# radiocosmology/driftscan

Measured on AMD Instinct MI355X. Metric: m-blocks/sec (BT-gen + SVD + KL), higher is better.
Workload: dtype f64; 1 GPU; configs[1]: 32-feed unpolarised cylinder, nfreq=16, nbase=46, lmax=mmax=128, 129 m-blocks per GPU per step, KLTransform with foregrounds; nfreq=16, nbase=46, lmax=128, mmax=128, sht_iter=3, mode=weak, ranks=1

## Files before the change

### driftscan_amd/_lib.py

```python
import ctypes
import os

import numpy as np

_HERE = os.path.dirname(os.path.abspath(__file__))
LIBPATH = os.path.join(_HERE, "lib", "libdriftmi.so")
if os.environ.get("DRIFTMI_LIB"):
    LIBPATH = os.environ["DRIFTMI_LIB"]

c_int = ctypes.c_int
c_i64 = ctypes.c_int64
c_dbl = ctypes.c_double
c_vp = ctypes.c_void_p
c_sz = ctypes.c_size_t

class ZgemmProblem(ctypes.Structure):
    _fields_ = [("A", c_vp), ("B", c_vp), ("C", c_vp), ("M", c_int), ("N", c_int), ("K", c_int),
                ("rsA", c_int), ("csA", c_int), ("rsB", c_int), ("csB", c_int), ("ldc", c_int),
                ("conjA", c_int), ("conjB", c_int), ("alpha", c_dbl), ("beta", c_dbl)]


class ZgemmProblemEx(ctypes.Structure):
    _fields_ = [("A", c_vp), ("B", c_vp), ("C", c_vp), ("kscale", c_vp), ("bgather", c_vp),
                ("M", c_int), ("N", c_int), ("K", c_int),
# ... 44 lines not shown
        c_int,
        [c_vp, c_int, c_int, c_int, c_dbl, c_vp, c_int, c_int, c_int, c_i64, c_vp, c_int, c_int, c_int, c_i64,
         c_dbl, c_vp, c_int, c_i64, c_vp, c_i64, c_int],
    ),
    "dm_zgemm_grouped": (c_int, [c_vp, c_int, ctypes.POINTER(ZgemmProblem)]),
    "dm_zgemm_grouped_ex": (c_int, [c_vp, c_int, ctypes.POINTER(ZgemmProblemEx)]),
    "dm_zgemm_plan_info": (c_int, [c_int, ctypes.POINTER(ZgemmProblemEx), c_int, ctypes.POINTER(ZgemmLaunchInfo),
                                   ctypes.POINTER(c_int)]),
    "dm_zpotrf_batched": (c_int, [c_vp, c_int, c_vp, c_int, c_i64, c_int, ctypes.POINTER(c_int)]),
    "dm_ztrsm_left_lower_batched": (
        c_int, [c_vp, c_int, c_int, c_vp, c_int, c_i64, c_vp, c_int, c_i64, c_int, c_int]),
    "dm_zpotrf_problems": (c_int, [c_vp, c_int, ctypes.POINTER(ZpotrfProblem), ctypes.POINTER(c_int)]),
    "dm_ztrsm_problems": (c_int, [c_vp, c_int, ctypes.POINTER(ZtrsmProblem), c_int, c_int]),
    "dm_zpotrf_problems_check": (c_int, [c_int, ctypes.POINTER(ZpotrfProblem)]),
    "dm_ztrsm_problems_check": (c_int, [c_int, ctypes.POINTER(ZtrsmProblem), c_int, c_int]),
    "dm_jacobi_rows_batched": (
        c_int, [c_vp, c_int, c_int, c_int, c_int, c_vp, c_int, c_i64, c_int, c_vp, ctypes.POINTER(c_int)]),
    "dm_jacobi_rows_problems": (
        c_int, [c_vp, c_int, ctypes.POINTER(JacobiProblemDesc), c_vp, c_int, ctypes.POINTER(JacobiOptions),
                ctypes.POINTER(c_int)]),
    "dm_jacobi_herm_batched": (
        c_int, [c_vp, c_int, c_vp, c_int, c_i64, c_vp, c_int, c_i64, c_int, c_vp, ctypes.POINTER(c_int)]),
    "dm_herm_eig_batched": (c_int, [c_vp, c_int, c_vp, c_int, c_i64, c_vp, c_int, c_i64, c_int, c_vp]),
    "dm_svd_chain": (
        c_int, [c_vp, c_int, c_int, c_int, c_int, c_int, c_vp, c_vp, c_dbl, c_vp, c_vp, c_vp, c_vp,
                ctypes.POINTER(c_int), ctypes.POINTER(c_int)]),
    "dm_svd_chain_lmin": (
        c_int, [c_vp, c_int, c_int, c_int, c_int, c_int, ctypes.POINTER(c_int), c_vp, c_vp, c_dbl, c_vp, c_vp, c_vp, c_vp,
                ctypes.POINTER(c_int), ctypes.POINTER(c_int)]),
    "dm_project_cov": (
# ... 392 lines not shown
        self.check(self.lib.dm_zpotrf_problems(self.h, n, _zpotrf_records(problems, ptrs), info), "dm_zpotrf_problems")
        return np.array(info[:n], dtype=np.int64)

    def ztrsm_problems(self, problems, conjtrans=False, upper_only=False):
        ptrs = []
        for p in problems:
            self._c128_device(p["L"], "ztrsm_problems")
            self._c128_device(p["B"], "ztrsm_problems")
            ztrsm_check_views(p, int(p["L"].numel()), int(p["B"].numel()))
            full = int(p["n"]) > 0 and int(p["nrhs"]) > 0
            ptrs.append((p["L"].data_ptr() + 16 * int(p.get("l_off", 0)) if full else 0,
                         p["B"].data_ptr() + 16 * int(p.get("b_off", 0)) if full else 0))
        self.check(self.lib.dm_ztrsm_problems(self.h, len(problems), _ztrsm_records(problems, ptrs),
                                              int(bool(conjtrans)), int(bool(upper_only))), "dm_ztrsm_problems")

    def jacobi_rows(self, Z, rows, cols, gc0, gc1, ld, stride=0, batch=1):
        sigma = self.empty((batch, max(rows, 1)), np.float64)
        sw = c_int(0)
        self.check(self.lib.dm_jacobi_rows_batched(self.h, rows, cols, gc0, gc1, self.ptr(Z), ld, stride, batch,
                                                   self.ptr(sigma), ctypes.byref(sw)), "dm_jacobi_rows_batched")
        return sigma, sw.value

    def jacobi_rows_problems(self, Z, problems, sigma=None, sigma_stride=None, **opts):
        n = len(problems)
        unknown = set(opts) - {f[0] for f in JacobiOptions._fields_}
        if unknown:
            raise ValueError("jacobi_rows_problems: unknown option(s) %s" % sorted(unknown))
        if n and not (Z.is_complex() and Z.element_size() == 16 and Z.is_contiguous()):
            raise ValueError("jacobi_rows_problems: a contiguous complex128 device tensor expected")
        arr = (JacobiProblemDesc * max(n, 1))()
# ... 1049 lines not shown
```

### driftscan_amd/csrc/dm_api.hip

```cpp
#include "dm_common.h"
#include "dm_kernels.h"
#include "../../include/driftmi.h"

#include <algorithm>

extern "C" {

int dm_zgemm_strided_batched(dm_ctx* ctx, int M, int N, int K, double alpha, const void* A, int rsA, int csA,
                             int conjA, int64_t strideA, const void* B, int rsB, int csB, int conjB,
                             int64_t strideB, double beta, void* C, int ldc, int64_t strideC,
                             const double* kscale, int64_t stride_kscale, int batch) {
  if (!ctx) return DM_EARG;
  DM_ARG(ctx, M >= 0 && N >= 0 && K >= 0 && batch >= 0 && A && B && C);
  dm_ws_scope ws_scope__(ctx);
  const size_t mark = ws_scope__.mark;
  std::vector<dm_gemm_desc> g;
  g.reserve(batch);
  for (int b = 0; b < batch; ++b) {
    g.push_back(dm_gemm_make(reinterpret_cast<const cplx*>(A) + b * strideA, rsA, csA, conjA != 0,
                             reinterpret_cast<const cplx*>(B) + b * strideB, rsB, csB, conjB != 0,
                             reinterpret_cast<cplx*>(C) + b * strideC, ldc, M, N, K, alpha, beta,
                             kscale ? kscale + b * stride_kscale : nullptr));
  }
  int rc = dm_gemm_grouped_launch(ctx, g);
// ... 189 lines not shown
  DM_TRY(dm_potrf_batched(ctx, mats, info_dev));
  return dm_download(ctx, info_host, info_dev, sizeof(int) * nprob);
}

int dm_ztrsm_problems(dm_ctx* ctx, int nprob, const dm_ztrsm_problem* probs, int conjtrans, int upper_only) {
  if (!ctx) return DM_EARG;
  DM_ARG(ctx, dm_ztrsm_problems_check(nprob, probs, conjtrans, upper_only) == DM_OK);
  dm_ws_scope ws_scope__(ctx);
  std::vector<dm_trsm_problem> ps(nprob);
  for (int i = 0; i < nprob; ++i)
    ps[i] = dm_trsm_problem{reinterpret_cast<const cplx*>(probs[i].L), probs[i].ldl, probs[i].n,
                            reinterpret_cast<cplx*>(probs[i].B), probs[i].ldb, probs[i].nrhs};
  return dm_trsm_left_lower_batched(ctx, ps, conjtrans != 0, upper_only != 0);
}

int dm_jacobi_rows_batched(dm_ctx* ctx, int rows, int cols, int gc0, int gc1, void* Z, int ld, int64_t stride,
                           int batch, double* sigma_dev, int* sweeps_host) {
  if (!ctx) return DM_EARG;
  DM_ARG(ctx, rows >= 0 && cols >= 0 && gc0 >= 0 && gc1 <= cols && gc0 <= gc1 && Z && sigma_dev && batch >= 0);
  std::vector<dm_jac_problem> ps(batch);
  for (int b = 0; b < batch; ++b)
    ps[b] = dm_jac_problem{reinterpret_cast<cplx*>(Z) + b * stride, ld, 0, rows, cols, gc0, gc1};
  return dm_jacobi_rows(ctx, ps, sigma_dev, rows > 0 ? rows : 1, sweeps_host);
}

int dm_jacobi_rows_problems(dm_ctx* ctx, int nprob, const dm_jacobi_problem_desc* probs, double* sigma_dev,
                            int sigma_stride, const dm_jacobi_options* opts, int* sweeps_host) {
  if (!ctx) return DM_EARG;
  DM_ARG(ctx, nprob >= 0 && (nprob == 0 || (probs && sigma_dev)) && sigma_stride >= 0);
  std::vector<dm_jac_problem> ps(nprob);
// ... 43 lines not shown
```

### driftscan_amd/csrc/dm_chol.hip

```cpp
#include "dm_common.h"
#include "dm_kernels.h"

#include <algorithm>

namespace {

constexpr int NB = 32;

struct chol_desc {
  cplx* A; int ld; int n;
};

__global__ __launch_bounds__(256) void potf2_kernel(const chol_desc* __restrict__ ds, int k0, int* __restrict__ info) {
  __shared__ cplx T[NB][NB + 1];
  __shared__ cplx Lo[NB][NB + 1];
  const chol_desc d = ds[blockIdx.x];
  if (k0 >= d.n) return;
  if (info[blockIdx.x] != 0) return;
  const int nb = min(NB, d.n - k0);
  const int tid = threadIdx.x;
  for (int idx = tid; idx < NB * NB; idx += 256) {
    int r = idx / NB, c = idx % NB;
    T[r][c] = (r < nb && c < nb && c <= r) ? d.A[(size_t)(k0 + r) * d.ld + k0 + c] : make_double2(0.0, 0.0);
    Lo[r][c] = make_double2(0.0, 0.0);
// ... 118 lines not shown
#pragma unroll
    for (int rr = 0; rr < NB; ++rr) {
      const int r = NB - 1 - rr;
      if (r < nb) {
        x[r] = cscale(x[r], 1.0 / Lk[r][r].x);
#pragma unroll
        for (int j = 0; j < r; ++j) x[j] = csub(x[j], cmul(cconj(Lk[r][j]), x[r]));
      }
    }
  }
#pragma unroll
  for (int r = 0; r < NB; ++r)
    if (r < nb) d.B[(size_t)(k0 + r) * d.ldb + col] = x[r];
}

}

int dm_potrf_batched(dm_ctx* ctx, const std::vector<dm_mat>& mats, int* info_dev) {
  const int nbatch = (int)mats.size();
  if (nbatch == 0) return DM_OK;
  dm_ws_scope ws_scope__(ctx);
  const size_t mark = ws_scope__.mark;
  std::vector<chol_desc> ds(nbatch);
  int maxn = 0;
  for (int i = 0; i < nbatch; ++i) {
    ds[i] = chol_desc{mats[i].p, mats[i].ld, mats[i].n};
    maxn = std::max(maxn, mats[i].n);
  }
  chol_desc* dd = dm_ws_upload(ctx, ds);
  if (!dd) return DM_ENOMEM;
  DM_HIP(ctx, hipMemsetAsync(info_dev, 0, sizeof(int) * nbatch, ctx->stream));
  if (maxn == 0) return DM_OK;
  dm_gemm_chain chain(ctx);
// ... 23 lines not shown
      const int k2 = k0 + 2 * NB;
      if (k2 < maxn) {
        DM_TRY(chain.gemm([&](std::vector<dm_gemm_desc>& g) {
          for (int i = 0; i < nbatch; ++i) {
            const int rem = mats[i].n - k2;
            if (rem <= 0) continue;
            cplx* L21 = mats[i].p + (size_t)k2 * mats[i].ld + k0;
            cplx* A22 = mats[i].p + (size_t)k2 * mats[i].ld + k2;
            g.push_back(dm_gemm_make(L21, mats[i].ld, 1, false, L21, 1, mats[i].ld, true, A22, mats[i].ld, rem, rem,
                                     2 * NB, -1.0, 1.0, nullptr, DM_GEMM_LOWER));
          }
        }));
      }
    }
  }
  DM_PLAUNCH(ctx, DM_PROF_CHOL, zero_upper_kernel, dim3((maxn + 255) / 256, maxn, nbatch), dim3(256), 0, ctx->stream, dd);
  DM_HIP(ctx, hipGetLastError());
  (void)mark;
  return DM_OK;
}

namespace {
int trsm_pass(dm_ctx* ctx, const std::vector<dm_trsm_problem>& probs, bool conjtrans, bool upper_only, dm_gemm_chain& chain,
              const trsm_desc* dd) {
  const int nbatch = (int)probs.size();
  int maxn = 0, maxrhs = 0;
  for (int i = 0; i < nbatch; ++i) {
    maxn = std::max(maxn, probs[i].n);
    maxrhs = std::max(maxrhs, probs[i].nrhs);
  }
  const int ct = (maxrhs + 255) / 256;
  const int NB2 = 2 * NB;
  const int nblk = (maxn + NB2 - 1) / NB2;
  const int nblk32 = (maxn + NB - 1) / NB;
  for (int s = 0; s < nblk; ++s) {
    DM_TRY(chain.gemm([&](std::vector<dm_gemm_desc>& g) {
    for (int i = 0; i < nbatch; ++i) {
      const dm_trsm_problem& P = probs[i];
      const int pn = (P.n + NB2 - 1) / NB2;
      if (!conjtrans) {
        if (s == 0 || s >= pn) continue;
        const int size = s & -s;
        const int r0 = s * NB2, r1 = std::min((s + size) * NB2, P.n);
        const int c0 = (s - size) * NB2;
        const int j0 = upper_only ? std::min(r0, P.nrhs) : 0;
        if (P.nrhs - j0 <= 0) continue;
        g.push_back(dm_gemm_make(P.L + (size_t)r0 * P.ldl + c0, P.ldl, 1, false, P.B + (size_t)c0 * P.ldb + j0, P.ldb, 1,
                                 false, P.B + (size_t)r0 * P.ldb + j0, P.ldb, r1 - r0, P.nrhs - j0, size * NB2, -1.0,
                                 1.0));
      } else {
        if (s < nblk - pn) continue;
        const int u = s - (nblk - pn);
        if (u == 0) continue;
        const int kb = pn - 1 - u;
        const int size = u & -u;
        const int t0 = std::max(kb - size + 1, 0) * NB2, t1 = (kb + 1) * NB2;
        const int k1 = t1, k2 = std::min((kb + 1 + size) * NB2, P.n);
        g.push_back(dm_gemm_make(P.L + (size_t)k1 * P.ldl + t0, 1, P.ldl, true, P.B + (size_t)k1 * P.ldb, P.ldb, 1,
                                 false, P.B + (size_t)t0 * P.ldb, P.ldb, t1 - t0, P.nrhs, k2 - k1, -1.0, 1.0));
      }
    }
    }));
    for (int half = 0; half < 2; ++half) {
      const int h = conjtrans ? 1 - half : half;
      int s32;
      if (!conjtrans) s32 = 2 * s + h;
      else s32 = 2 * s + half;
      if (chain.dry) {
      } else if (!conjtrans)
        DM_PLAUNCH(ctx, DM_PROF_CHOL, diag_solve_kernel<false>, dim3(ct, nbatch), dim3(256), 0, ctx->stream, dd, s32, nblk32,
                           upper_only ? 1 : 0);
      else
        DM_PLAUNCH(ctx, DM_PROF_CHOL, diag_solve_kernel<true>, dim3(ct, nbatch), dim3(256), 0, ctx->stream, dd, s32, 2 * nblk, 0);
      if (half == 0) {
        DM_TRY(chain.gemm([&](std::vector<dm_gemm_desc>& g2) {
        for (int i = 0; i < nbatch; ++i) {
          const dm_trsm_problem& P = probs[i];
          const int pn = (P.n + NB2 - 1) / NB2;
          if (!conjtrans) {
            const int k0 = s * NB2, k1 = k0 + NB;
            if (k1 >= P.n) continue;
            const int nb = std::min(NB, P.n - k1);
            const int j0 = upper_only ? std::min(k0, P.nrhs) : 0;
            if (P.nrhs - j0 <= 0) continue;
            g2.push_back(dm_gemm_make(P.L + (size_t)k1 * P.ldl + k0, P.ldl, 1, false, P.B + (size_t)k0 * P.ldb + j0,
                                      P.ldb, 1, false, P.B + (size_t)k1 * P.ldb + j0, P.ldb, nb, P.nrhs - j0, NB, -1.0,
                                      1.0));
          } else {
            if (s < nblk - pn) continue;
            const int kb = pn - 1 - (s - (nblk - pn));
            const int k0 = kb * NB2, k1 = k0 + NB;
            if (k1 >= P.n) continue;
            const int nb2 = std::min(NB, P.n - k1);
            g2.push_back(dm_gemm_make(P.L + (size_t)k1 * P.ldl + k0, 1, P.ldl, true, P.B + (size_t)k1 * P.ldb, P.ldb,
                                      1, false, P.B + (size_t)k0 * P.ldb, P.ldb, NB, P.nrhs, nb2, -1.0, 1.0));
          }
        }
        }));
      }
    }
  }
  return DM_OK;
}
}

int dm_trsm_plan_build(dm_ctx* ctx, const std::vector<dm_trsm_problem>& probs, bool conjtrans, bool upper_only, dm_trsm_plan& plan) {
  if (conjtrans) upper_only = false;
  if (upper_only)
    for (const auto& P : probs) DM_ARG(ctx, P.nrhs == P.n);
  plan.probs = probs;
  plan.conjtrans = conjtrans;
  plan.upper_only = upper_only;
  plan.chain.reset(new dm_gemm_chain(ctx));
  plan.empty = true;
  for (const auto& P : probs)
    if (P.n > 0 && P.nrhs > 0) plan.empty = false;
  if (plan.empty) return DM_OK;
  return trsm_pass(ctx, plan.probs, conjtrans, upper_only, *plan.chain, nullptr);
}

int dm_trsm_plan_run(dm_ctx* ctx, dm_trsm_plan& plan) {
  if (plan.empty || !plan.chain) return DM_OK;
  const int nbatch = (int)plan.probs.size();
  std::vector<trsm_desc> ds(nbatch);
  for (int i = 0; i < nbatch; ++i)
    ds[i] = trsm_desc{plan.probs[i].L, plan.probs[i].ldl, plan.probs[i].n, plan.probs[i].B, plan.probs[i].ldb, plan.probs[i].nrhs};
  trsm_desc* dd = dm_ws_upload(ctx, ds);
  if (!dd) return DM_ENOMEM;
  DM_TRY(plan.chain->upload());
  DM_TRY(trsm_pass(ctx, plan.probs, plan.conjtrans, plan.upper_only, *plan.chain, dd));
  DM_HIP(ctx, hipGetLastError());
  return DM_OK;
}

int dm_trsm_left_lower_batched(dm_ctx* ctx, const std::vector<dm_trsm_problem>& probs, bool conjtrans, bool upper_only) {
  dm_trsm_plan plan;
  DM_TRY(dm_trsm_plan_build(ctx, probs, conjtrans, upper_only, plan));
  return dm_trsm_plan_run(ctx, plan);
}
```

### driftscan_amd/csrc/dm_kernels.h

```cpp
#pragma once

#include "dm_common.h"

#include <deque>
#include <memory>
#include <functional>

enum {
  DM_GEMM_CONJ_A = 1,
  DM_GEMM_CONJ_B = 2,
  DM_GEMM_B_REAL = 4,
  DM_GEMM_LOWER = 8,
  DM_GEMM_ALL_REAL = 16,
  DM_GEMM_UPPER = 32,
  DM_GEMM_UPPER128 = 128,
  DM_GEMM_B_GATHER = 64,
};

struct dm_gemm_desc {
  const void* A;
  const void* B;
  void* C;
  const double* kscale;
  const int2* bgather;
// ... 95 lines not shown
                   int* sweeps_out = nullptr);

struct dm_eig_select {
  std::function<void(int p, const double* ev, int n, std::vector<int>& cols)> pick;
  std::vector<int> nsel;
};
int dm_herm_eig_tridiag(dm_ctx* ctx, const std::vector<dm_jac_herm_problem>& probs, double* evals, int evals_stride,
                        dm_eig_select* sel = nullptr, int two_stage = -1);

int dm_sort_rows_by_key(dm_ctx* ctx, const std::vector<dm_jac_problem>& probs, double* key, int key_stride,
                        bool descending);

struct dm_mat {
  cplx* p; int ld; int n;
};
int dm_potrf_batched(dm_ctx* ctx, const std::vector<dm_mat>& mats, int* info_dev);
struct dm_trsm_problem {
  const cplx* L; int ldl; int n;
  cplx* B; int ldb; int nrhs;
};
int dm_trsm_left_lower_batched(dm_ctx* ctx, const std::vector<dm_trsm_problem>& probs, bool conjtrans, bool upper_only = false);
struct dm_gemm_chain;
struct dm_trsm_plan {
  std::vector<dm_trsm_problem> probs;
  bool conjtrans = false, upper_only = false, empty = true;
  std::shared_ptr<dm_gemm_chain> chain;
};
int dm_trsm_plan_build(dm_ctx* ctx, const std::vector<dm_trsm_problem>& probs, bool conjtrans, bool upper_only, dm_trsm_plan& plan);
int dm_trsm_plan_run(dm_ctx* ctx, dm_trsm_plan& plan);

constexpr int DM_BAND_LC = 4;

struct dm_band_proj {
  int nblk = 0, F = 0, K = 0, P = 0, L = 0, R = 0;
  const int* svnum = nullptr;
  const int* nmodes = nullptr;
  const int64_t* evals_off = nullptr;
  std::vector<int> ndof, active, l0eff;
  std::vector<int64_t> off1;
  size_t tot1 = 0, totw = 0;
  int init(dm_ctx* ctx, int nblk_, int F_, int K_, int P_, int L_, const int* svnum_host, const int* l0_host,
           const int* nmodes_host, const int64_t* evals_off_host, int R_);
  int to_svd(dm_ctx* ctx, const cplx* evecs, const int64_t* evecs_off, const double* w, const int64_t* x_off, int nset,
// ... 21 lines not shown
```

### driftscan_amd/csrc/dm_kl.hip

```cpp
#include "dm_common.h"
#include "dm_kernels.h"
#include "../../include/driftmi.h"

#include <algorithm>
#include <chrono>
#include <cmath>

namespace {

struct blk_desc {
  cplx* a; int n;
};

constexpr int BLK_SPLIT = 16;

__device__ __forceinline__ bool lex_gt(double are, double aim, double bre, double bim) {
  return are > bre || (are == bre && aim > bim);
}

__global__ __launch_bounds__(256) void lexmax_partial_kernel(const blk_desc* __restrict__ bd, double2* __restrict__ part) {
  const blk_desc d = bd[blockIdx.y];
  __shared__ double sre[256], sim[256];
  double bre = -INFINITY, bim = -INFINITY;
  const size_t tot = (size_t)d.n * d.n;
// ... 43 lines not shown
  const size_t tot = (size_t)d.n * d.n;
  int mine = 0;
  for (size_t i = (size_t)blockIdx.x * 256 + threadIdx.x; i < tot; i += (size_t)BLK_SPLIT * 256) {
    cplx v = d.a[i];
    if (v.x != 0.0 || v.y != 0.0) mine = 1;
  }
  if (mine) flag[blockIdx.y] = 0;
}

__global__ void add_diag_kernel(const blk_desc* __restrict__ bd, const double* __restrict__ val) {
  const blk_desc d = bd[blockIdx.y];
  const int i = blockIdx.x * blockDim.x + threadIdx.x;
  if (i < d.n) d.a[(size_t)i * d.n + i].x += val[blockIdx.y];
}


int copy_async(dm_ctx* ctx, cplx* dst, const cplx* src, size_t n) {
  if (n == 0) return DM_OK;
  DM_HIP(ctx, hipMemcpyAsync(dst, src, n * sizeof(cplx), hipMemcpyDeviceToDevice, ctx->stream));
  return DM_OK;
}

}

extern "C" {

int dm_project_cov(dm_ctx* ctx, int nblk, int F, int K, int P, int L, const void* beam_svd_dev,
                   const int* svnum_host, const int* l0_host, const double* cl_pfl_dev, int npol,
                   const int* polmask_host, void* out_dev, const int64_t* out_off_host, int zero_first) {
  if (!ctx) return DM_EARG;
// ... 148 lines not shown
  cplx* E = reinterpret_cast<cplx*>(evecs_dev);

  size_t tot = 0;
  int maxn = 0;
  for (int b = 0; b < nblk; ++b) {
    tot += (size_t)n_host[b] * n_host[b];
    maxn = std::max(maxn, n_host[b]);
    add_const_host[b] = 0.0;
  }
  std::vector<size_t> loff(nblk);
  {
    size_t o = 0;
    for (int b = 0; b < nblk; ++b) { loff[b] = o; o += (size_t)n_host[b] * n_host[b]; }
  }
  cplx* Lw = dm_ws_alloc_t<cplx>(ctx, std::max<size_t>(tot, 1));
  cplx* Tw = dm_ws_alloc_t<cplx>(ctx, std::max<size_t>(tot, 1));
  cplx* Ww = dm_ws_alloc_t<cplx>(ctx, std::max<size_t>(tot, 1));
  double* evw = dm_ws_alloc_t<double>(ctx, (size_t)nblk * std::max(maxn, 1));
  int* info_dev = dm_ws_alloc_t<int>(ctx, nblk);
  int* zflag_dev = dm_ws_alloc_t<int>(ctx, nblk);
  if (!Lw || !Tw || !Ww || !evw || !info_dev || !zflag_dev) return DM_ENOMEM;

  std::vector<blk_desc> bdA(nblk);
  for (int b = 0; b < nblk; ++b) bdA[b] = blk_desc{A + off_host[b], n_host[b]};
  blk_desc* d_bdA = dm_ws_upload(ctx, bdA);
  if (!d_bdA) return DM_ENOMEM;
  DM_PLAUNCH(ctx, DM_PROF_UTIL, flag_set_kernel, dim3((nblk + 255) / 256), dim3(256), 0, ctx->stream, zflag_dev, nblk, 1);
  DM_PLAUNCH(ctx, DM_PROF_UTIL, allzero_kernel, dim3(BLK_SPLIT, nblk), dim3(256), 0, ctx->stream, d_bdA, zflag_dev);
  auto factor_launch = [&](const std::vector<int>& blks) -> int {
    std::vector<dm_mat> mats;
    std::vector<dm_cdesc> cp;
    for (int b : blks) {
      cp.push_back(dm_cdesc{B + off_host[b], Lw + loff[b], sizeof(cplx) * (size_t)n_host[b] * n_host[b]});
      mats.push_back(dm_mat{Lw + loff[b], n_host[b], n_host[b]});
    }
    DM_TRY(dm_copy_batched(ctx, cp));
    return dm_potrf_batched(ctx, mats, info_dev);
  };
  auto factor = [&](const std::vector<int>& blks, std::vector<int>& info) -> int {
    DM_TRY(factor_launch(blks));
    info.resize(blks.size());
    if (!blks.empty()) DM_TRY(dm_download(ctx, info.data(), info_dev, sizeof(int) * blks.size()));
    return DM_OK;
  };
  auto trsm_lists = [&](const std::vector<int>& blks, std::vector<dm_trsm_problem>& t1, std::vector<dm_trsm_problem>& t2) {
    t1.clear();
    t2.clear();
    for (int b : blks) {
      t1.push_back(dm_trsm_problem{Lw + loff[b], n_host[b], n_host[b], A + off_host[b], n_host[b], n_host[b]});
      t2.push_back(dm_trsm_problem{Lw + loff[b], n_host[b], n_host[b], Tw + loff[b], n_host[b], n_host[b]});
    }
  };
  std::vector<int> cand;
  for (int b = 0; b < nblk; ++b)
    if (n_host[b] > 0) cand.push_back(b);
  static const bool host_times = getenv("DM_TIME_HOST") != nullptr;
  const auto ht0 = std::chrono::steady_clock::now();
  DM_TRY(factor_launch(cand));
  const auto ht1 = std::chrono::steady_clock::now();
  dm_trsm_plan plan1, plan2;
  {
    std::vector<dm_trsm_problem> t1, t2;
    trsm_lists(cand, t1, t2);
    DM_TRY(dm_trsm_plan_build(ctx, t1, false, false, plan1));
    DM_TRY(dm_trsm_plan_build(ctx, t2, false, true, plan2));
  }
  const auto ht2 = std::chrono::steady_clock::now();
  std::vector<int> zflag(nblk);
  DM_TRY(dm_download(ctx, zflag.data(), zflag_dev, sizeof(int) * nblk));
  if (host_times) {
    const auto ht3 = std::chrono::steady_clock::now();
    auto ms = [](auto a, auto b) { return std::chrono::duration<double, std::milli>(b - a).count(); };
    fprintf(stderr, "HOSTTIME eigh_gen: potrf plan+launch %.3f ms, trsm plans %.3f ms, wait for flags %.3f ms\n", ms(ht0, ht1),
            ms(ht1, ht2), ms(ht2, ht3));
  }
  std::vector<int> info_c(cand.size());
  if (!cand.empty()) DM_TRY(dm_download(ctx, info_c.data(), info_dev, sizeof(int) * cand.size()));

  std::vector<int> work;
// ... 3 lines not shown
    if (zflag[b]) {
      DM_TRY(dm_fill_zero(ctx, evals_dev + evoff_host[b], sizeof(double) * n_host[b]));
      DM_TRY(dm_set_identity(ctx, E + off_host[b], n_host[b], n_host[b]));
      if (nkeep_host && cut_mode) {
        const int cut = 0.0 >= cut_value ? 0 : n_host[b];
        nkeep_host[b] = cut_mode == 1 ? n_host[b] - cut : cut;
      }
    } else {
      work.push_back(b);
      info.push_back(info_c[i]);
    }
  }
  if (work.size() != cand.size()) {
    std::vector<dm_trsm_problem> t1, t2;
    trsm_lists(work, t1, t2);
    DM_TRY(dm_trsm_plan_build(ctx, t1, false, false, plan1));
    DM_TRY(dm_trsm_plan_build(ctx, t2, false, true, plan2));
  }
  std::vector<int> bad;
  for (size_t i = 0; i < work.size(); ++i)
    if (info[i] != 0) bad.push_back(work[i]);
  if (!bad.empty()) {
    std::vector<dm_jac_herm_problem> hp;
    for (int b : bad) {
      DM_TRY(copy_async(ctx, Tw + loff[b], B + off_host[b], (size_t)n_host[b] * n_host[b]));
      DM_TRY(dm_hermitize(ctx, Tw + loff[b], n_host[b], n_host[b]));
      hp.push_back(dm_jac_herm_problem{Tw + loff[b], n_host[b], Ww + loff[b], n_host[b], n_host[b]});
    }
    DM_TRY(dm_herm_eig_tridiag(ctx, hp, evw, std::max(maxn, 1)));
    std::vector<double> hev((size_t)bad.size() * std::max(maxn, 1));
    DM_TRY(dm_download(ctx, hev.data(), evw, sizeof(double) * hev.size()));
    std::vector<double> shifts(nblk, 0.0);
    for (size_t i = 0; i < bad.size(); ++i) {
      const int b = bad[i];
      const double* ev = &hev[i * std::max(maxn, 1)];
      double mn = ev[0], mx = ev[0];
      for (int k = 1; k < n_host[b]; ++k) { mn = std::min(mn, ev[k]); mx = std::max(mx, ev[k]); }
// ... 11 lines not shown
    if (!d_bdB || !d_sh) return DM_ENOMEM;
    DM_PLAUNCH(ctx, DM_PROF_UTIL, add_diag_kernel, dim3((maxn + 255) / 256, (unsigned)bad.size()), dim3(256), 0, ctx->stream,
                       d_bdB, d_sh);
    std::vector<int> info2;
    DM_TRY(factor(bad, info2));
    for (size_t i = 0; i < bad.size(); ++i)
      if (info2[i] != 0) {
        ctx->err = "dm_eigh_gen: B is not positive definite even after the diagonal rescue";
        dm_ws_release(ctx, mark);
        return info2[i];
      }
  }

  {
    DM_TRY(dm_trsm_plan_run(ctx, plan1));
    std::vector<dm_tdesc> tr;
    for (int b : work) tr.push_back(dm_tdesc{A + off_host[b], n_host[b], Tw + loff[b], n_host[b], n_host[b], n_host[b]});
    DM_TRY(dm_conj_transpose_batched(ctx, tr));
    DM_TRY(dm_trsm_plan_run(ctx, plan2));
  }

  std::vector<int> i_ev(nblk, 0);
  std::vector<std::vector<double>> evsorted(nblk);
  {
    std::vector<dm_jac_herm_problem> hp;
    for (int b : work) hp.push_back(dm_jac_herm_problem{Tw + loff[b], n_host[b], Ww + loff[b], n_host[b], n_host[b]});
    dm_eig_select sel;
    sel.pick = [&](int p, const double* ev, int n, std::vector<int>& cols) {
      const int b = work[p];
      std::vector<int> order(n);
      for (int i = 0; i < n; ++i) order[i] = i;
      std::stable_sort(order.begin(), order.end(), [&](int x, int y) { return ev[x] < ev[y]; });
      evsorted[b].resize(n);
      for (int i = 0; i < n; ++i) evsorted[b][i] = ev[order[i]];
      const int cut = (int)(std::lower_bound(evsorted[b].begin(), evsorted[b].end(), cut_value) - evsorted[b].begin());
      i_ev[b] = cut;
      if (cut_mode == 1) cols.assign(order.begin() + cut, order.end());
      else if (cut_mode == 2) cols.assign(order.begin(), order.begin() + cut);
      else cols = order;
    };
    DM_TRY(dm_herm_eig_tridiag(ctx, hp, evw, std::max(maxn, 1), &sel));
// ... 1 lines not shown
    for (size_t i = 0; i + 1 < work.size() && contiguous; ++i)
      contiguous = evoff_host[work[i + 1]] == evoff_host[work[i]] + n_host[work[i]];
    if (contiguous) {
      std::vector<double> flat;
      for (int b : work) flat.insert(flat.end(), evsorted[b].begin(), evsorted[b].end());
      DM_TRY(dm_upload(ctx, evals_dev + evoff_host[work.front()], flat.data(), sizeof(double) * flat.size()));
    }
    for (size_t i = 0; i < work.size(); ++i) {
      const int b = work[i];
      if (nkeep_host) nkeep_host[b] = sel.nsel[i];
      if (!contiguous)
        DM_TRY(dm_upload(ctx, evals_dev + evoff_host[b], evsorted[b].data(), sizeof(double) * n_host[b]));
    }
  }

  {
    std::vector<dm_trsm_problem> t3;
    std::vector<dm_tdesc> tr1, tr2;
    bool span_ok = cut_mode != 0 && !work.empty();
    for (size_t i = 0; i + 1 < work.size() && span_ok; ++i)
      span_ok = off_host[work[i + 1]] == off_host[work[i]] + (int64_t)n_host[work[i]] * n_host[work[i]];
    if (span_ok) {
      const int bl = work.back();
      DM_TRY(dm_fill_zero(ctx, E + off_host[work.front()],
                          sizeof(cplx) * (size_t)(off_host[bl] + (int64_t)n_host[bl] * n_host[bl] - off_host[work.front()])));
    }
    for (size_t i = 0; i < work.size(); ++i) {
      const int b = work[i];
      const int n = n_host[b];
      const int nk = cut_mode == 1 ? n - i_ev[b] : (cut_mode == 2 ? i_ev[b] : n);
      const int row0 = cut_mode == 1 ? i_ev[b] : 0;
      if (nk < n && !span_ok) DM_TRY(dm_fill_zero(ctx, E + off_host[b], sizeof(cplx) * (size_t)n * n));
      if (nk <= 0) continue;
      tr1.push_back(dm_tdesc{Ww + loff[b], n, Tw + loff[b], nk, nk, n});
      t3.push_back(dm_trsm_problem{Lw + loff[b], n, n, Tw + loff[b], nk, nk});
      tr2.push_back(dm_tdesc{Tw + loff[b], nk, E + off_host[b] + (size_t)row0 * n, n, n, nk});
    }
    DM_TRY(dm_conj_transpose_batched(ctx, tr1));
    DM_TRY(dm_trsm_left_lower_batched(ctx, t3, true));
    DM_TRY(dm_conj_transpose_batched(ctx, tr2));
  }
  DM_HIP(ctx, hipStreamSynchronize(ctx->stream));
  dm_ws_release(ctx, mark);
  return DM_OK;
}


static int kl_covariances(dm_ctx* ctx, int nblk, int F, int K, int P, int L, int T, const void* beam_svd_dev,
                          const void* beam_ut_dev, const int* svnum_host, const int* l0_host, const double* cl_sg_dev,
                          const int* sg_mask_host, int sg_symmetric, const double* cl_fg_dev, const int* fg_mask_host,
                          int fg_symmetric, const double* npower_dev, double noise_scale, double regulariser,
                          const std::vector<int>& ndof, const std::vector<int64_t>& off, cplx* S, cplx* N) {
  DM_TRY(dm_project_cov(ctx, nblk, F, K, P, L, beam_svd_dev, svnum_host, l0_host, cl_sg_dev, P, sg_mask_host, S, off.data(),
                        1 | (sg_symmetric ? 2 : 0)));
  if (cl_fg_dev) {
// ... 146 lines not shown
```

### include/driftmi.h

```cpp
#ifndef DRIFTMI_H
#define DRIFTMI_H

#include <stddef.h>
#include <stdint.h>

#ifdef __cplusplus
extern "C" {
#endif

typedef struct dm_ctx dm_ctx;

int dm_ctx_create(int device, size_t workspace_bytes, void* stream, dm_ctx** out);
int dm_ctx_destroy(dm_ctx* ctx);
int dm_ctx_sync(dm_ctx* ctx);
size_t dm_ctx_workspace_bytes(dm_ctx* ctx);
int dm_ctx_workspace_reset(dm_ctx* ctx, size_t bytes);
const char* dm_last_error(dm_ctx* ctx);
int dm_version(void);

int dm_prof_trd_stride(void);

int dm_prof_reset(dm_ctx* ctx, int enable);
int dm_prof_report(dm_ctx* ctx, double* ms, double* flops, long long* launches);

// ... 56 lines not shown

typedef struct dm_zpotrf_problem {
  void* A;
  int n, ld;
} dm_zpotrf_problem;
int dm_zpotrf_problems(dm_ctx* ctx, int nprob, const dm_zpotrf_problem* probs_host, int* info_host);

typedef struct dm_ztrsm_problem {
  const void* L;
  int ldl, n;
  void* B;
  int ldb, nrhs;
} dm_ztrsm_problem;
int dm_ztrsm_problems(dm_ctx* ctx, int nprob, const dm_ztrsm_problem* probs_host, int conjtrans, int upper_only);

int dm_zpotrf_problems_check(int nprob, const dm_zpotrf_problem* probs_host);
int dm_ztrsm_problems_check(int nprob, const dm_ztrsm_problem* probs_host, int conjtrans, int upper_only);

int dm_jacobi_rows_batched(dm_ctx* ctx, int rows, int cols, int gc0, int gc1, void* Z_dev, int ld, int64_t stride,
                           int batch, double* sigma_dev, int* sweeps_host);

typedef struct dm_jacobi_problem_desc {
  void* Z;
  int ld, row0, nrows, ncols, gc0, gc1;
} dm_jacobi_problem_desc;
typedef struct dm_jacobi_options {
  int unconverged;
  double drop_below;
  int one_stage_eig;
  double subspace_cut;
// ... 175 lines not shown
```

Baseline: 1157 m-blocks/s.

## Add right-side batched TRSM to drop conjugate-transposes in generalized eigensolve

Adds a right-side lower-triangular batched TRSM (new diagonal-solve kernel plus GEMM updates), so the KL generalized eigenproblem solves in place instead of transposing into a temporary. The first L^-1 A L^-H step and the final back-transform now avoid several conjugate-transpose passes and the Tw workspace. The Cholesky input copy is reduced to a lower-triangle copy without zeroing the upper part, and a single kernel places eigenvector rows and zero-fills E. The cost is a new solve path whose diagonal kernel tiles 64 rows per block with a serial per-row solve, which may use the GPU less efficiently than the existing left-side kernel.

```diff
diff --git a/driftscan_amd/_lib.py b/driftscan_amd/_lib.py
--- a/driftscan_amd/_lib.py
+++ b/driftscan_amd/_lib.py
@@ -82,6 +82,8 @@
     "dm_ztrsm_problems": (c_int, [c_vp, c_int, ctypes.POINTER(ZtrsmProblem), c_int, c_int]),
     "dm_zpotrf_problems_check": (c_int, [c_int, ctypes.POINTER(ZpotrfProblem)]),
     "dm_ztrsm_problems_check": (c_int, [c_int, ctypes.POINTER(ZtrsmProblem), c_int, c_int]),
+    "dm_ztrsm_right_problems": (c_int, [c_vp, c_int, ctypes.POINTER(ZtrsmProblem), c_int]),
+    "dm_ztrsm_right_problems_check": (c_int, [c_int, ctypes.POINTER(ZtrsmProblem)]),
     "dm_jacobi_rows_batched": (
         c_int, [c_vp, c_int, c_int, c_int, c_int, c_vp, c_int, c_i64, c_int, c_vp, ctypes.POINTER(c_int)]),
     "dm_jacobi_rows_problems": (
@@ -504,6 +506,24 @@
         self.check(self.lib.dm_ztrsm_problems(self.h, len(problems), _ztrsm_records(problems, ptrs),
                                               int(bool(conjtrans)), int(bool(upper_only))), "dm_ztrsm_problems")
 
+    def ztrsm_right_problems(self, problems, conjtrans=False):
+        ptrs = []
+        for p in problems:
+            self._c128_device(p["L"], "ztrsm_right_problems")
+            self._c128_device(p["B"], "ztrsm_right_problems")
+            n, nrhs, ldl, ldb = (int(p[k]) for k in ("n", "nrhs", "ldl", "ldb"))
+            l_off, b_off = int(p.get("l_off", 0)), int(p.get("b_off", 0))
+            if min(n, nrhs, ldl, ldb, l_off, b_off) < 0:
+                raise ValueError("ztrsm_right_problems: negative size, leading dimension or offset")
+            full = n > 0 and nrhs > 0
+            if full and l_off + (n - 1) * ldl + n > int(p["L"].numel()):
+                raise ValueError("ztrsm_right_problems: L reaches outside its tensor")
+            if full and b_off + (nrhs - 1) * ldb + n > int(p["B"].numel()):
+                raise ValueError("ztrsm_right_problems: B reaches outside its tensor")
+            ptrs.append((p["L"].data_ptr() + 16 * l_off if full else 0, p["B"].data_ptr() + 16 * b_off if full else 0))
+        self.check(self.lib.dm_ztrsm_right_problems(self.h, len(problems), _ztrsm_records(problems, ptrs),
+                                                    int(bool(conjtrans))), "dm_ztrsm_right_problems")
+
     def jacobi_rows(self, Z, rows, cols, gc0, gc1, ld, stride=0, batch=1):
         sigma = self.empty((batch, max(rows, 1)), np.float64)
         sw = c_int(0)
diff --git a/driftscan_amd/csrc/dm_api.hip b/driftscan_amd/csrc/dm_api.hip
--- a/driftscan_amd/csrc/dm_api.hip
+++ b/driftscan_amd/csrc/dm_api.hip
@@ -227,6 +227,28 @@
   return dm_trsm_left_lower_batched(ctx, ps, conjtrans != 0, upper_only != 0);
 }
 
+int dm_ztrsm_right_problems_check(int nprob, const dm_ztrsm_problem* probs) {
+  if (nprob < 0 || (nprob > 0 && !probs)) return DM_EARG;
+  for (int i = 0; i < nprob; ++i) {
+    const dm_ztrsm_problem& p = probs[i];
+    if (p.n < 0 || p.nrhs < 0 || p.ldl < 0 || p.ldb < 0) return DM_EARG;
+    if (p.n > 0 && (p.ldl < p.n || p.ldb < p.n)) return DM_EARG;
+    if (p.n > 0 && p.nrhs > 0 && (!p.L || !p.B)) return DM_EARG;
+  }
+  return DM_OK;
+}
+
+int dm_ztrsm_right_problems(dm_ctx* ctx, int nprob, const dm_ztrsm_problem* probs, int conjtrans) {
+  if (!ctx) return DM_EARG;
+  DM_ARG(ctx, dm_ztrsm_right_problems_check(nprob, probs) == DM_OK);
+  dm_ws_scope ws_scope__(ctx);
+  std::vector<dm_trsm_problem> ps(nprob);
+  for (int i = 0; i < nprob; ++i)
+    ps[i] = dm_trsm_problem{reinterpret_cast<const cplx*>(probs[i].L), probs[i].ldl, probs[i].n,
+                            reinterpret_cast<cplx*>(probs[i].B), probs[i].ldb, probs[i].nrhs};
+  return dm_trsm_right_lower_batched(ctx, ps, conjtrans != 0);
+}
+
 int dm_jacobi_rows_batched(dm_ctx* ctx, int rows, int cols, int gc0, int gc1, void* Z, int ld, int64_t stride,
                            int batch, double* sigma_dev, int* sweeps_host) {
   if (!ctx) return DM_EARG;
diff --git a/driftscan_amd/csrc/dm_chol.hip b/driftscan_amd/csrc/dm_chol.hip
--- a/driftscan_amd/csrc/dm_chol.hip
+++ b/driftscan_amd/csrc/dm_chol.hip
@@ -156,9 +156,71 @@
     if (r < nb) d.B[(size_t)(k0 + r) * d.ldb + col] = x[r];
 }
 
-}
-
-int dm_potrf_batched(dm_ctx* ctx, const std::vector<dm_mat>& mats, int* info_dev) {
+template <bool CONJTRANS>
+__global__ __launch_bounds__(256) void diag_solve_right_kernel(const trsm_desc* __restrict__ ds, int s, int nblk) {
+  __shared__ cplx Lk[NB][NB + 1];
+  __shared__ cplx R[64][NB + 1];
+  const trsm_desc d = ds[blockIdx.y];
+  int k0;
+  if (CONJTRANS) {
+    k0 = s * NB;
+  } else {
+    const int pn = (d.n + NB - 1) / NB;
+    if (s < nblk - pn) return;
+    k0 = (pn - 1 - (s - (nblk - pn))) * NB;
+  }
+  if (k0 >= d.n || k0 < 0) return;
+  const int r0 = blockIdx.x * 64;
+  if (r0 >= d.nrhs) return;
+  const int nb = min(NB, d.n - k0);
+  const int tid = threadIdx.x;
+  for (int idx = tid; idx < NB * NB; idx += 256) {
+    int r = idx / NB, c = idx % NB;
+    Lk[r][c] = (r < nb && c < nb) ? d.L[(size_t)(k0 + r) * d.ldl + k0 + c] : make_double2(0.0, 0.0);
+  }
+  for (int idx = tid; idx < 64 * NB; idx += 256) {
+    int r = idx / NB, c = idx % NB;
+    R[r][c] = (r0 + r < d.nrhs && c < nb) ? d.B[(size_t)(r0 + r) * d.ldb + k0 + c] : make_double2(0.0, 0.0);
+  }
+  __syncthreads();
+  if (tid < 64) {
+    const int r = tid;
+    cplx x[NB];
+#pragma unroll
+    for (int c = 0; c < NB; ++c) x[c] = R[r][c];
+    if (CONJTRANS) {
+#pragma unroll
+      for (int c = 0; c < NB; ++c) {
+        if (c < nb) {
+          x[c] = cscale(x[c], 1.0 / Lk[c][c].x);
+#pragma unroll
+          for (int j = c + 1; j < NB; ++j) x[j] = csub(x[j], cmulc(x[c], Lk[j][c]));
+        }
+      }
+    } else {
+#pragma unroll
+      for (int cc = 0; cc < NB; ++cc) {
+        const int c = NB - 1 - cc;
+        if (c < nb) {
+          x[c] = cscale(x[c], 1.0 / Lk[c][c].x);
+#pragma unroll
+          for (int j = 0; j < c; ++j) x[j] = csub(x[j], cmul(x[c], Lk[c][j]));
+        }
+      }
+    }
+#pragma unroll
+    for (int c = 0; c < NB; ++c) R[r][c] = x[c];
+  }
+  __syncthreads();
+  for (int idx = tid; idx < 64 * NB; idx += 256) {
+    int r = idx / NB, c = idx % NB;
+    if (r0 + r < d.nrhs && c < nb) d.B[(size_t)(r0 + r) * d.ldb + k0 + c] = R[r][c];
+  }
+}
+
+}
+
+int dm_potrf_batched(dm_ctx* ctx, const std::vector<dm_mat>& mats, int* info_dev, bool zero_upper) {
   const int nbatch = (int)mats.size();
   if (nbatch == 0) return DM_OK;
   dm_ws_scope ws_scope__(ctx);
@@ -212,40 +274,58 @@
       }
     }
   }
-  DM_PLAUNCH(ctx, DM_PROF_CHOL, zero_upper_kernel, dim3((maxn + 255) / 256, maxn, nbatch), dim3(256), 0, ctx->stream, dd);
+  if (zero_upper)
+    DM_PLAUNCH(ctx, DM_PROF_CHOL, zero_upper_kernel, dim3((maxn + 255) / 256, maxn, nbatch), dim3(256), 0, ctx->stream, dd);
   DM_HIP(ctx, hipGetLastError());
   (void)mark;
   return DM_OK;
 }
 
 namespace {
-int trsm_pass(dm_ctx* ctx, const std::vector<dm_trsm_problem>& probs, bool conjtrans, bool upper_only, dm_gemm_chain& chain,
-              const trsm_desc* dd) {
+int trsm_pass(dm_ctx* ctx, const std::vector<dm_trsm_problem>& probs, bool right, bool conjtrans, bool upper_only,
+              dm_gemm_chain& chain, const trsm_desc* dd) {
   const int nbatch = (int)probs.size();
   int maxn = 0, maxrhs = 0;
   for (int i = 0; i < nbatch; ++i) {
     maxn = std::max(maxn, probs[i].n);
     maxrhs = std::max(maxrhs, probs[i].nrhs);
   }
-  const int ct = (maxrhs + 255) / 256;
+  const bool fwd = right ? conjtrans : !conjtrans;
+  const int ct = right ? (maxrhs + 63) / 64 : (maxrhs + 255) / 256;
   const int NB2 = 2 * NB;
   const int nblk = (maxn + NB2 - 1) / NB2;
   const int nblk32 = (maxn + NB - 1) / NB;
+  auto update = [&](std::vector<dm_gemm_desc>& g, const dm_trsm_problem& P, int t0, int t1, int k1, int k2, int j0) {
+    if (!right) {
+      if (!conjtrans)
+        g.push_back(dm_gemm_make(P.L + (size_t)t0 * P.ldl + k1, P.ldl, 1, false, P.B + (size_t)k1 * P.ldb + j0, P.ldb, 1,
+                                 false, P.B + (size_t)t0 * P.ldb + j0, P.ldb, t1 - t0, P.nrhs - j0, k2 - k1, -1.0, 1.0));
+      else
+        g.push_back(dm_gemm_make(P.L + (size_t)k1 * P.ldl + t0, 1, P.ldl, true, P.B + (size_t)k1 * P.ldb + j0, P.ldb, 1,
+                                 false, P.B + (size_t)t0 * P.ldb + j0, P.ldb, t1 - t0, P.nrhs - j0, k2 - k1, -1.0, 1.0));
+    } else {
+      if (P.nrhs <= 0) return;
+      if (conjtrans)
+        g.push_back(dm_gemm_make(P.B + k1, P.ldb, 1, false, P.L + (size_t)t0 * P.ldl + k1, 1, P.ldl, true, P.B + t0, P.ldb,
+                                 P.nrhs, t1 - t0, k2 - k1, -1.0, 1.0));
+      else
+        g.push_back(dm_gemm_make(P.B + k1, P.ldb, 1, false, P.L + (size_t)k1 * P.ldl + t0, P.ldl, 1, false, P.B + t0, P.ldb,
+                                 P.nrhs, t1 - t0, k2 - k1, -1.0, 1.0));
+    }
+  };
   for (int s = 0; s < nblk; ++s) {
     DM_TRY(chain.gemm([&](std::vector<dm_gemm_desc>& g) {
     for (int i = 0; i < nbatch; ++i) {
       const dm_trsm_problem& P = probs[i];
       const int pn = (P.n + NB2 - 1) / NB2;
-      if (!conjtrans) {
+      if (fwd) {
         if (s == 0 || s >= pn) continue;
         const int size = s & -s;
         const int r0 = s * NB2, r1 = std::min((s + size) * NB2, P.n);
         const int c0 = (s - size) * NB2;
         const int j0 = upper_only ? std::min(r0, P.nrhs) : 0;
         if (P.nrhs - j0 <= 0) continue;
-        g.push_back(dm_gemm_make(P.L + (size_t)r0 * P.ldl + c0, P.ldl, 1, false, P.B + (size_t)c0 * P.ldb + j0, P.ldb, 1,
-                                 false, P.B + (size_t)r0 * P.ldb + j0, P.ldb, r1 - r0, P.nrhs - j0, size * NB2, -1.0,
-                                 1.0));
+        update(g, P, r0, r1, c0, r0, j0);
       } else {
         if (s < nblk - pn) continue;
         const int u = s - (nblk - pn);
@@ -254,17 +334,22 @@
         const int size = u & -u;
         const int t0 = std::max(kb - size + 1, 0) * NB2, t1 = (kb + 1) * NB2;
         const int k1 = t1, k2 = std::min((kb + 1 + size) * NB2, P.n);
-        g.push_back(dm_gemm_make(P.L + (size_t)k1 * P.ldl + t0, 1, P.ldl, true, P.B + (size_t)k1 * P.ldb, P.ldb, 1,
-                                 false, P.B + (size_t)t0 * P.ldb, P.ldb, t1 - t0, P.nrhs, k2 - k1, -1.0, 1.0));
+        update(g, P, t0, t1, k1, k2, 0);
       }
     }
     }));
     for (int half = 0; half < 2; ++half) {
-      const int h = conjtrans ? 1 - half : half;
+      const int h = fwd ? half : 1 - half;
       int s32;
-      if (!conjtrans) s32 = 2 * s + h;
+      if (fwd) s32 = 2 * s + h;
       else s32 = 2 * s + half;
       if (chain.dry) {
+      } else if (right) {
+        if (conjtrans)
+          DM_PLAUNCH(ctx, DM_PROF_CHOL, diag_solve_right_kernel<true>, dim3(ct, nbatch), dim3(256), 0, ctx->stream, dd, s32, nblk32);
+        else
+          DM_PLAUNCH(ctx, DM_PROF_CHOL, diag_solve_right_kernel<false>, dim3(ct, nbatch), dim3(256), 0, ctx->stream, dd, s32,
+                             2 * nblk);
       } else if (!conjtrans)
         DM_PLAUNCH(ctx, DM_PROF_CHOL, diag_solve_kernel<false>, dim3(ct, nbatch), dim3(256), 0, ctx->stream, dd, s32, nblk32,
                            upper_only ? 1 : 0);
@@ -275,23 +360,20 @@
         for (int i = 0; i < nbatch; ++i) {
           const dm_trsm_problem& P = probs[i];
           const int pn = (P.n + NB2 - 1) / NB2;
-          if (!conjtrans) {
+          if (fwd) {
             const int k0 = s * NB2, k1 = k0 + NB;
             if (k1 >= P.n) continue;
             const int nb = std::min(NB, P.n - k1);
             const int j0 = upper_only ? std::min(k0, P.nrhs) : 0;
             if (P.nrhs - j0 <= 0) continue;
-            g2.push_back(dm_gemm_make(P.L + (size_t)k1 * P.ldl + k0, P.ldl, 1, false, P.B + (size_t)k0 * P.ldb + j0,
-                                      P.ldb, 1, false, P.B + (size_t)k1 * P.ldb + j0, P.ldb, nb, P.nrhs - j0, NB, -1.0,
-                                      1.0));
+            update(g2, P, k1, k1 + nb, k0, k1, j0);
           } else {
             if (s < nblk - pn) continue;
             const int kb = pn - 1 - (s - (nblk - pn));
             const int k0 = kb * NB2, k1 = k0 + NB;
             if (k1 >= P.n) continue;
             const int nb2 = std::min(NB, P.n - k1);
-            g2.push_back(dm_gemm_make(P.L + (size_t)k1 * P.ldl + k0, 1, P.ldl, true, P.B + (size_t)k1 * P.ldb, P.ldb,
-                                      1, false, P.B + (size_t)k0 * P.ldb, P.ldb, NB, P.nrhs, nb2, -1.0, 1.0));
+            update(g2, P, k0, k1, k1, k1 + nb2, 0);
           }
         }
         }));
@@ -302,19 +384,22 @@
 }
 }
 
-int dm_trsm_plan_build(dm_ctx* ctx, const std::vector<dm_trsm_problem>& probs, bool conjtrans, bool upper_only, dm_trsm_plan& plan) {
+int dm_trsm_plan_build(dm_ctx* ctx, const std::vector<dm_trsm_problem>& probs, bool conjtrans, bool upper_only, dm_trsm_plan& plan,
+                       bool right) {
   if (conjtrans) upper_only = false;
+  DM_ARG(ctx, !(right && upper_only));
   if (upper_only)
     for (const auto& P : probs) DM_ARG(ctx, P.nrhs == P.n);
   plan.probs = probs;
   plan.conjtrans = conjtrans;
   plan.upper_only = upper_only;
+  plan.right = right;
   plan.chain.reset(new dm_gemm_chain(ctx));
   plan.empty = true;
   for (const auto& P : probs)
     if (P.n > 0 && P.nrhs > 0) plan.empty = false;
   if (plan.empty) return DM_OK;
-  return trsm_pass(ctx, plan.probs, conjtrans, upper_only, *plan.chain, nullptr);
+  return trsm_pass(ctx, plan.probs, right, conjtrans, upper_only, *plan.chain, nullptr);
 }
 
 int dm_trsm_plan_run(dm_ctx* ctx, dm_trsm_plan& plan) {
@@ -326,7 +411,7 @@
   trsm_desc* dd = dm_ws_upload(ctx, ds);
   if (!dd) return DM_ENOMEM;
   DM_TRY(plan.chain->upload());
-  DM_TRY(trsm_pass(ctx, plan.probs, plan.conjtrans, plan.upper_only, *plan.chain, dd));
+  DM_TRY(trsm_pass(ctx, plan.probs, plan.right, plan.conjtrans, plan.upper_only, *plan.chain, dd));
   DM_HIP(ctx, hipGetLastError());
   return DM_OK;
 }
@@ -336,3 +421,9 @@
   DM_TRY(dm_trsm_plan_build(ctx, probs, conjtrans, upper_only, plan));
   return dm_trsm_plan_run(ctx, plan);
 }
+
+int dm_trsm_right_lower_batched(dm_ctx* ctx, const std::vector<dm_trsm_problem>& probs, bool conjtrans) {
+  dm_trsm_plan plan;
+  DM_TRY(dm_trsm_plan_build(ctx, probs, conjtrans, false, plan, true));
+  return dm_trsm_plan_run(ctx, plan);
+}
diff --git a/driftscan_amd/csrc/dm_kernels.h b/driftscan_amd/csrc/dm_kernels.h
--- a/driftscan_amd/csrc/dm_kernels.h
+++ b/driftscan_amd/csrc/dm_kernels.h
@@ -133,19 +133,21 @@
 struct dm_mat {
   cplx* p; int ld; int n;
 };
-int dm_potrf_batched(dm_ctx* ctx, const std::vector<dm_mat>& mats, int* info_dev);
+int dm_potrf_batched(dm_ctx* ctx, const std::vector<dm_mat>& mats, int* info_dev, bool zero_upper = true);
 struct dm_trsm_problem {
   const cplx* L; int ldl; int n;
   cplx* B; int ldb; int nrhs;
 };
 int dm_trsm_left_lower_batched(dm_ctx* ctx, const std::vector<dm_trsm_problem>& probs, bool conjtrans, bool upper_only = false);
+int dm_trsm_right_lower_batched(dm_ctx* ctx, const std::vector<dm_trsm_problem>& probs, bool conjtrans);
 struct dm_gemm_chain;
 struct dm_trsm_plan {
   std::vector<dm_trsm_problem> probs;
-  bool conjtrans = false, upper_only = false, empty = true;
+  bool conjtrans = false, upper_only = false, empty = true, right = false;
   std::shared_ptr<dm_gemm_chain> chain;
 };
-int dm_trsm_plan_build(dm_ctx* ctx, const std::vector<dm_trsm_problem>& probs, bool conjtrans, bool upper_only, dm_trsm_plan& plan);
+int dm_trsm_plan_build(dm_ctx* ctx, const std::vector<dm_trsm_problem>& probs, bool conjtrans, bool upper_only, dm_trsm_plan& plan,
+                       bool right = false);
 int dm_trsm_plan_run(dm_ctx* ctx, dm_trsm_plan& plan);
 
 constexpr int DM_BAND_LC = 4;
diff --git a/driftscan_amd/csrc/dm_kl.hip b/driftscan_amd/csrc/dm_kl.hip
--- a/driftscan_amd/csrc/dm_kl.hip
+++ b/driftscan_amd/csrc/dm_kl.hip
@@ -81,6 +81,33 @@
   if (i < d.n) d.a[(size_t)i * d.n + i].x += val[blockIdx.y];
 }
 
+struct tril_desc {
+  const cplx* src; cplx* dst; int n;
+};
+__global__ __launch_bounds__(256) void tril_copy_kernel(const tril_desc* __restrict__ ds) {
+  const tril_desc d = ds[blockIdx.y];
+  const int r = blockIdx.x;
+  if (r >= d.n) return;
+  const cplx* s = d.src + (size_t)r * d.n;
+  cplx* t = d.dst + (size_t)r * d.n;
+  for (int c = threadIdx.x; c <= r; c += 256) t[c] = s[c];
+}
+
+struct place_desc {
+  const cplx* W; cplx* E; int n; int row0; int nk;
+};
+__global__ __launch_bounds__(256) void place_rows_kernel(const place_desc* __restrict__ ds) {
+  const place_desc d = ds[blockIdx.y];
+  const int r = blockIdx.x;
+  if (r >= d.n) return;
+  cplx* t = d.E + (size_t)r * d.n;
+  if (r >= d.row0 && r < d.row0 + d.nk) {
+    const cplx* s = d.W + (size_t)(r - d.row0) * d.n;
+    for (int c = threadIdx.x; c < d.n; c += 256) t[c] = s[c];
+  } else {
+    for (int c = threadIdx.x; c < d.n; c += 256) t[c] = make_double2(0.0, 0.0);
+  }
+}
 
 int copy_async(dm_ctx* ctx, cplx* dst, const cplx* src, size_t n) {
   if (n == 0) return DM_OK;
@@ -259,12 +286,11 @@
     for (int b = 0; b < nblk; ++b) { loff[b] = o; o += (size_t)n_host[b] * n_host[b]; }
   }
   cplx* Lw = dm_ws_alloc_t<cplx>(ctx, std::max<size_t>(tot, 1));
-  cplx* Tw = dm_ws_alloc_t<cplx>(ctx, std::max<size_t>(tot, 1));
   cplx* Ww = dm_ws_alloc_t<cplx>(ctx, std::max<size_t>(tot, 1));
   double* evw = dm_ws_alloc_t<double>(ctx, (size_t)nblk * std::max(maxn, 1));
   int* info_dev = dm_ws_alloc_t<int>(ctx, nblk);
   int* zflag_dev = dm_ws_alloc_t<int>(ctx, nblk);
-  if (!Lw || !Tw || !Ww || !evw || !info_dev || !zflag_dev) return DM_ENOMEM;
+  if (!Lw || !Ww || !evw || !info_dev || !zflag_dev) return DM_ENOMEM;
 
   std::vector<blk_desc> bdA(nblk);
   for (int b = 0; b < nblk; ++b) bdA[b] = blk_desc{A + off_host[b], n_host[b]};
@@ -274,13 +300,19 @@
   DM_PLAUNCH(ctx, DM_PROF_UTIL, allzero_kernel, dim3(BLK_SPLIT, nblk), dim3(256), 0, ctx->stream, d_bdA, zflag_dev);
   auto factor_launch = [&](const std::vector<int>& blks) -> int {
     std::vector<dm_mat> mats;
-    std::vector<dm_cdesc> cp;
+    std::vector<tril_desc> cp;
+    int mn = 0;
     for (int b : blks) {
-      cp.push_back(dm_cdesc{B + off_host[b], Lw + loff[b], sizeof(cplx) * (size_t)n_host[b] * n_host[b]});
+      cp.push_back(tril_desc{B + off_host[b], Lw + loff[b], n_host[b]});
       mats.push_back(dm_mat{Lw + loff[b], n_host[b], n_host[b]});
-    }
-    DM_TRY(dm_copy_batched(ctx, cp));
-    return dm_potrf_batched(ctx, mats, info_dev);
+      mn = std::max(mn, n_host[b]);
+    }
+    if (mn > 0) {
+      tril_desc* d_cp = dm_ws_upload(ctx, cp);
+      if (!d_cp) return DM_ENOMEM;
+      DM_PLAUNCH(ctx, DM_PROF_UTIL, tril_copy_kernel, dim3(mn, (unsigned)cp.size()), dim3(256), 0, ctx->stream, d_cp);
+    }
+    return dm_potrf_batched(ctx, mats, info_dev, false);
   };
   auto factor = [&](const std::vector<int>& blks, std::vector<int>& info) -> int {
     DM_TRY(factor_launch(blks));
@@ -293,7 +325,7 @@
     t2.clear();
     for (int b : blks) {
       t1.push_back(dm_trsm_problem{Lw + loff[b], n_host[b], n_host[b], A + off_host[b], n_host[b], n_host[b]});
-      t2.push_back(dm_trsm_problem{Lw + loff[b], n_host[b], n_host[b], Tw + loff[b], n_host[b], n_host[b]});
+      t2.push_back(t1.back());
     }
   };
   std::vector<int> cand;
@@ -307,7 +339,7 @@
   {
     std::vector<dm_trsm_problem> t1, t2;
     trsm_lists(cand, t1, t2);
-    DM_TRY(dm_trsm_plan_build(ctx, t1, false, false, plan1));
+    DM_TRY(dm_trsm_plan_build(ctx, t1, true, false, plan1, true));
     DM_TRY(dm_trsm_plan_build(ctx, t2, false, true, plan2));
   }
   const auto ht2 = std::chrono::steady_clock::now();
@@ -341,13 +373,15 @@
   if (work.size() != cand.size()) {
     std::vector<dm_trsm_problem> t1, t2;
     trsm_lists(work, t1, t2);
-    DM_TRY(dm_trsm_plan_build(ctx, t1, false, false, plan1));
+    DM_TRY(dm_trsm_plan_build(ctx, t1, true, false, plan1, true));
     DM_TRY(dm_trsm_plan_build(ctx, t2, false, true, plan2));
   }
   std::vector<int> bad;
   for (size_t i = 0; i < work.size(); ++i)
     if (info[i] != 0) bad.push_back(work[i]);
   if (!bad.empty()) {
+    cplx* Tw = dm_ws_alloc_t<cplx>(ctx, std::max<size_t>(tot, 1));
+    if (!Tw) return DM_ENOMEM;
     std::vector<dm_jac_herm_problem> hp;
     for (int b : bad) {
       DM_TRY(copy_async(ctx, Tw + loff[b], B + off_host[b], (size_t)n_host[b] * n_host[b]));
@@ -389,9 +423,6 @@
 
   {
     DM_TRY(dm_trsm_plan_run(ctx, plan1));
-    std::vector<dm_tdesc> tr;
-    for (int b : work) tr.push_back(dm_tdesc{A + off_host[b], n_host[b], Tw + loff[b], n_host[b], n_host[b], n_host[b]});
-    DM_TRY(dm_conj_transpose_batched(ctx, tr));
     DM_TRY(dm_trsm_plan_run(ctx, plan2));
   }
 
@@ -399,7 +430,7 @@
   std::vector<std::vector<double>> evsorted(nblk);
   {
     std::vector<dm_jac_herm_problem> hp;
-    for (int b : work) hp.push_back(dm_jac_herm_problem{Tw + loff[b], n_host[b], Ww + loff[b], n_host[b], n_host[b]});
+    for (int b : work) hp.push_back(dm_jac_herm_problem{A + off_host[b], n_host[b], Ww + loff[b], n_host[b], n_host[b]});
     dm_eig_select sel;
     sel.pick = [&](int p, const double* ev, int n, std::vector<int>& cols) {
       const int b = work[p];
@@ -431,31 +462,23 @@
     }
   }
 
-  {
+  if (!work.empty()) {
     std::vector<dm_trsm_problem> t3;
-    std::vector<dm_tdesc> tr1, tr2;
-    bool span_ok = cut_mode != 0 && !work.empty();
-    for (size_t i = 0; i + 1 < work.size() && span_ok; ++i)
-      span_ok = off_host[work[i + 1]] == off_host[work[i]] + (int64_t)n_host[work[i]] * n_host[work[i]];
-    if (span_ok) {
-      const int bl = work.back();
-      DM_TRY(dm_fill_zero(ctx, E + off_host[work.front()],
-                          sizeof(cplx) * (size_t)(off_host[bl] + (int64_t)n_host[bl] * n_host[bl] - off_host[work.front()])));
-    }
+    std::vector<place_desc> pl;
+    int mn = 0;
     for (size_t i = 0; i < work.size(); ++i) {
       const int b = work[i];
       const int n = n_host[b];
-      const int nk = cut_mode == 1 ? n - i_ev[b] : (cut_mode == 2 ? i_ev[b] : n);
+      const int nk = std::max(cut_mode == 1 ? n - i_ev[b] : (cut_mode == 2 ? i_ev[b] : n), 0);
       const int row0 = cut_mode == 1 ? i_ev[b] : 0;
-      if (nk < n && !span_ok) DM_TRY(dm_fill_zero(ctx, E + off_host[b], sizeof(cplx) * (size_t)n * n));
-      if (nk <= 0) continue;
-      tr1.push_back(dm_tdesc{Ww + loff[b], n, Tw + loff[b], nk, nk, n});
-      t3.push_back(dm_trsm_problem{Lw + loff[b], n, n, Tw + loff[b], nk, nk});
-      tr2.push_back(dm_tdesc{Tw + loff[b], nk, E + off_host[b] + (size_t)row0 * n, n, n, nk});
-    }
-    DM_TRY(dm_conj_transpose_batched(ctx, tr1));
-    DM_TRY(dm_trsm_left_lower_batched(ctx, t3, true));
-    DM_TRY(dm_conj_transpose_batched(ctx, tr2));
+      pl.push_back(place_desc{Ww + loff[b], E + off_host[b], n, row0, nk});
+      mn = std::max(mn, n);
+      if (nk > 0) t3.push_back(dm_trsm_problem{Lw + loff[b], n, n, E + off_host[b] + (size_t)row0 * n, n, nk});
+    }
+    place_desc* d_pl = dm_ws_upload(ctx, pl);
+    if (!d_pl) return DM_ENOMEM;
+    DM_PLAUNCH(ctx, DM_PROF_UTIL, place_rows_kernel, dim3(mn, (unsigned)pl.size()), dim3(256), 0, ctx->stream, d_pl);
+    DM_TRY(dm_trsm_right_lower_batched(ctx, t3, false));
   }
   DM_HIP(ctx, hipStreamSynchronize(ctx->stream));
   dm_ws_release(ctx, mark);
diff --git a/include/driftmi.h b/include/driftmi.h
--- a/include/driftmi.h
+++ b/include/driftmi.h
@@ -94,6 +94,9 @@
 } dm_ztrsm_problem;
 int dm_ztrsm_problems(dm_ctx* ctx, int nprob, const dm_ztrsm_problem* probs_host, int conjtrans, int upper_only);
 
+int dm_ztrsm_right_problems(dm_ctx* ctx, int nprob, const dm_ztrsm_problem* probs_host, int conjtrans);
+int dm_ztrsm_right_problems_check(int nprob, const dm_ztrsm_problem* probs_host);
+
 int dm_zpotrf_problems_check(int nprob, const dm_zpotrf_problem* probs_host);
 int dm_ztrsm_problems_check(int nprob, const dm_ztrsm_problem* probs_host, int conjtrans, int upper_only);
 
```

Result: no change. 1164 m-blocks/s (median of 6 runs) (+0.6%).
